# alibaba/EasyRec

Hardware: AMD Instinct MI355X
Metric: global examples/sec + emb HBM GB/s, DeepFM Criteo-shape b4096 @1/2/4/8 GPU (higher is better)
Workload: dtype f32; 1 GPU; DeepFM synthetic Criteo: deepfm_criteo.config (39 features: 26 hashed x 1000000 rows + 13 projected, D=16 deep + D=1 wide, batch 4096 per GPU, optimizer adam_optimizer (lazy dense decay, closed-form replay), ids zipf, hipGraph replay); timed steps cycle over 256 distinct device-generated batches after 1024 untimed pre-conditioning steps; global_batch=4096, parallelism=single GPU

## Files before the change

### easyrec_amd/csrc/er_embedding.hip

```cpp
#include <algorithm>
#include <cmath>
#include <cstring>
#include <vector>

#include "er_common.h"
#include "er_gemm_core.h"
#include "er_dense_tail.h"
#include "er_decay.h"
#include "er_grad_finish.h"

namespace er {

constexpr uint32_t kInvalidKey = 0xFFFFFFFFu;

__host__ __device__ __forceinline__ void lane_geom(int dim, int& V, int& G) {
  V = (dim % 4 == 0) ? 4 : 1;
  const int n = dim / V;
  G = 1;
  while (G < n) G <<= 1;
}

__device__ __forceinline__ int find_lookup(const int32_t* __restrict__ blk_start, int n, int bid) {
  int lo = 0, hi = n;
  while (hi - lo > 1) {
// ... 1266 lines not shown
  float* s_all = smem;
  for (int i = tid; i < kProjParts * (dim + 1); i += kBlock)
    s_all[i] = __hip_atomic_load(all + i, __ATOMIC_RELAXED, __HIP_MEMORY_SCOPE_SYSTEM);
  __syncthreads();
  if (tid >= G || !col_ok) return;
  float g[V];
#pragma unroll
  for (int j = 0; j < V; ++j) g[j] = 0.f;
  float n_valid = 0.f;
  for (int k = 0; k < kProjParts; ++k) {
#pragma unroll
    for (int j = 0; j < V; ++j) g[j] = g[j] + s_all[k * (dim + 1) + c + j];
    n_valid = n_valid + s_all[k * (dim + 1) + dim];
  }
  if (n_valid == 0.f) return;
  const ReduceOut ro{0, nullptr, nullptr, nullptr, nullptr, 0};
  finish_run<V>(a.tab, ma.opt_kind, ma.hyper, ro, static_cast<uint32_t>(d.key_base), 0, sub, c, dim, g, a.aux);
  if (dbg && tid == 0) dbg[1] = wall_clock64();
}

#ifndef ER_OWN_WAVES
#define ER_OWN_WAVES 4
#endif
__device__ __forceinline__ void own_block(int bid, const OwnMulti& ma, float* smem) {
  if (bid < ma.start[ma.n]) {
    int i = 0;
    while (i + 1 < ma.n && bid >= ma.start[i + 1]) ++i;
    const OwnArgs& a = ma.a[i];
    if (a.V == 4) own_tile_body<4>(bid - ma.start[i], ma, a, smem);
    else own_tile_body<1>(bid - ma.start[i], ma, a, smem);
    return;
  }
  const int pb = bid - ma.start[ma.n];
  int i = 0;
  while (i + 1 < ma.n && pb >= ma.proj_start[i + 1]) ++i;
  const OwnArgs& a = ma.a[i];
  if (a.V == 4) own_proj_body<4>(pb - ma.proj_start[i], ma, a, smem);
  else own_proj_body<1>(pb - ma.proj_start[i], ma, a, smem);
}

__global__ void __launch_bounds__(kBlock) __attribute__((amdgpu_waves_per_eu(ER_OWN_WAVES)))
emb_bwd_own_kernel(OwnMulti ma) {
  extern __shared__ __attribute__((aligned(16))) float smem[];
  own_block(blockIdx.x, ma, smem);
}

__global__ void __launch_bounds__(kBlock) __attribute__((amdgpu_waves_per_eu(ER_OWN_WAVES)))
emb_bwd_own_wgrad_kernel(OwnMulti ma, GroupedArgs ga, int n_gemm, int n_own, LossTailArgs lt) {
  extern __shared__ __attribute__((aligned(16))) float smem[];
  const int bid = blockIdx.x;
  if (bid < n_gemm) {
    const GroupedCoords c = grouped_coords(ga, bid);
    if (c.split < 0) return;
    gemm_f32_block<false, false>(ga.p[c.p], c.tile, c.split, smem, c.plain);
    return;
  }
  if (bid - n_gemm < n_own) own_block(bid - n_gemm, ma, smem);
  else loss_tail_body<kBlock>(lt, smem);
}

struct CatchHeadsArgs {
  const uint32_t* ukeys_seg;
  const uint32_t* seg_count;
  const int64_t* ent_base;
  int n_lookups;
  int64_t n;
  RowUpdate tab;
  DecayAux aux;
  int dim, G, V;
  const uint32_t* extra_keys;
  int n_extra;
  int cap_shift;
};
struct CatchHeadsMulti {
  int n;
  int start[kMaxMulti + 1];
  const er_opt_hyper* hyper;
  CatchHeadsArgs a[kMaxMulti];
};

template <int V>
__device__ __forceinline__ void catch_up_row(const CatchHeadsArgs& a, uint32_t key, int c, int32_t t, float eps) {
  const int32_t s_begin = a.tab.ls(key) + 1;
  if (s_begin >= t) return;
  const int64_t off = a.tab.off(key, c);
  float var[V], m[V], v[V];
  ld_vec<V>(m, a.tab.m + off);
  ld_vec<V>(v, a.tab.v + off);
  bool live = false;
#pragma unroll
  for (int j = 0; j < V; ++j) live = live || (m[j] != 0.f) || (v[j] != 0.f);
  if (live) {
    ld_vec<V>(var, a.tab.var + off);
    replay_closed<V>(var, m, v, a.aux, s_begin, t, eps);
    st_vec<V>(a.tab.var + off, var);
    st_vec<V>(a.tab.m + off, m);
    st_vec<V>(a.tab.v + off, v);
  }
  if (c == 0) a.tab.ls(key) = t - 1;
}

template <int V>
__device__ __forceinline__ void catch_heads_body(int bid, const CatchHeadsArgs& a, const er_opt_hyper* __restrict__ hyper) {
  __shared__ int s_base[kOwnMaxLookups + 1], s_cnt[kOwnMaxLookups + 1];
  const int tid = threadIdx.x;
  const int ppb = kBlock / a.G;
  const int c = (tid % a.G) * V;
// ... 3408 lines not shown
```

### easyrec_amd/csrc/er_gemm.hip

```cpp
#include "er_gemm_core.h"

namespace er {

template <bool A_KC, bool B_KC>
__global__ void __launch_bounds__(kBlock)
gemm_f32_kernel(GemmArgs g) {
  __shared__ __attribute__((aligned(16))) float lds[2 * 2 * kOpTile];
  gemm_f32_block<A_KC, B_KC>(g, blockIdx.x, blockIdx.z, lds);
}

template <bool A_KC, bool B_KC>
__global__ void __launch_bounds__(kBlock)
gemm_f32_bn_bwd_kernel(GemmArgs g) {
  __shared__ __attribute__((aligned(16))) float lds[2 * 2 * kOpTile];
  gemm_f32_block<A_KC, B_KC, true>(g, blockIdx.x, 0, lds);
}

template <bool A_KC, bool B_KC, int XEPI>
__global__ void __launch_bounds__(kBlock)
gemm_f32_cross_kernel(GemmArgs g, er_gemm_epilogue xe) {
  __shared__ __attribute__((aligned(16))) float lds[2 * 2 * kOpTile];
  gemm_f32_block<A_KC, B_KC, false, XEPI>(g, blockIdx.x, 0, lds, false, &xe);
}

template <bool A_KC, bool B_KC, int DIN>
__global__ void __launch_bounds__(kBlock)
gemm_f32_din_kernel(GemmArgs g, DinGen d) {
  __shared__ __attribute__((aligned(16))) float lds[2 * 2 * kOpTile];
  gemm_f32_block<A_KC, B_KC, false, 0, DIN>(g, blockIdx.x, blockIdx.z, lds, false, nullptr, &d);
}

__global__ void __launch_bounds__(kBlock)
gemm_f32_bna_kernel(GemmArgs g, BnA b) {
  __shared__ __attribute__((aligned(16))) float lds[2 * 2 * kOpTile];
  __shared__ __attribute__((aligned(16))) float coef[4 * kBnAMaxK];
  bna_load_coef(b, g.K, coef);
  __syncthreads();
  gemm_f32_block<true, false, false, 0, 3>(g, blockIdx.x, 0, lds, false, nullptr, nullptr, &b, coef);
}

template <int NC>
__global__ void __launch_bounds__(kBlock)
gemv_bna_kernel(const float* __restrict__ x, int ldx, int M, int K, BnA b, const float* __restrict__ W, int ldw,
                const float* __restrict__ bias, float* __restrict__ C, int ldc, int lpr) {
  constexpr int R = 4;
  const int rpb = kBlock / lpr;
  const int lr = threadIdx.x % lpr;
  const int r0 = (static_cast<int>(blockIdx.x) * R) * rpb + threadIdx.x / lpr;
  const bool bn = b.mean != nullptr;
  float acc[R][NC];
#pragma unroll
  for (int u = 0; u < R; ++u)
#pragma unroll
    for (int n = 0; n < NC; ++n) acc[u][n] = 0.f;
  for (int c = lr; c < K / 4; c += lpr) {
    const int k = 4 * c;
    f32x4v xv[R];
#pragma unroll
    for (int u = 0; u < R; ++u) {
      int row = r0 + u * rpb;
      row = row < M ? row : M - 1;
      xv[u] = *reinterpret_cast<const f32x4v*>(x + static_cast<int64_t>(row) * ldx + k);
    }
    float w[4][NC];
#pragma unroll
    for (int j = 0; j < 4; ++j)
#pragma unroll
      for (int n = 0; n < NC; ++n) w[j][n] = W[static_cast<int64_t>(k + j) * ldw + n];
// ... 309 lines not shown
  __shared__ __attribute__((aligned(16))) short Bs[BN * kBf16SH];
  const GroupedCoords c = grouped_coords(ga, blockIdx.x);
  if (c.split < 0) return;
  gemm_bf16_block<A_KC, B_KC>(ga.p[c.p], c.tile, c.split, As, Bs, c.plain);
}


template <int VEC>
__global__ void __launch_bounds__(kBlock)
gemm_splitk_reduce_kernel(const float* __restrict__ ws, int64_t mn, int N, int splits, const float* __restrict__ bias,
                          float* __restrict__ C, int ldc, int accumulate) {
  splitk_reduce_elems<VEC>(ws, mn, N, splits, bias, C, ldc, accumulate,
                           (static_cast<int64_t>(blockIdx.x) * kBlock + threadIdx.x) * VEC);
}


template <int VEC>
__global__ void __launch_bounds__(kBlock)
gemm_splitk_reduce_grouped_kernel(GroupedReduceArgs ra) {
  splitk_reduce_grouped_block<VEC>(ra, blockIdx.x);
}

}

namespace {

float* g_gemm_ws = nullptr;
size_t g_gemm_ws_floats = 0;

int ensure_ws(size_t floats, float** out) {
  if (floats > g_gemm_ws_floats) {
    if (g_gemm_ws) (void)hipFree(g_gemm_ws);
    g_gemm_ws = nullptr;
    g_gemm_ws_floats = 0;
    ER_CHECK_HIP(hipMalloc(&g_gemm_ws, floats * sizeof(float)));
    g_gemm_ws_floats = floats;
  }
  *out = g_gemm_ws;
  return 0;
}

template <bool BF16>
int launch_gemm(int layout, er::GemmArgs& a, hipStream_t s) {
  const int64_t n_tiles = er::ceil_div(a.N, er::BN) * er::ceil_div(a.M, er::BM);
  dim3 grid(static_cast<unsigned>(n_tiles), 1, static_cast<unsigned>(a.splits));
  dim3 block(er::kBlock);
#define ER_LAUNCH_GEMM(KERNEL)                                                   \
  switch (layout) {                                                              \
    case ER_GEMM_NN: hipLaunchKernelGGL((KERNEL<true, false>), grid, block, 0, s, a); break;  \
    case ER_GEMM_NT: hipLaunchKernelGGL((KERNEL<true, true>), grid, block, 0, s, a); break;   \
    case ER_GEMM_TN: hipLaunchKernelGGL((KERNEL<false, false>), grid, block, 0, s, a); break; \
    default: er::set_error("er_gemm: unknown layout %d", layout); return 2;     \
  }
  if (BF16) {
    ER_LAUNCH_GEMM(er::gemm_bf16_kernel)
  } else if (a.bn.partial) {
    ER_LAUNCH_GEMM(er::gemm_f32_bn_bwd_kernel)
  } else {
    ER_LAUNCH_GEMM(er::gemm_f32_kernel)
  }
#undef ER_LAUNCH_GEMM
  ER_LAUNCH_CHECK();
  return 0;
}

int choose_splits(int M, int N, int K, int ktile) {
  const int64_t tiles = er::ceil_div(M, er::BM) * er::ceil_div(N, er::BN);
  if (tiles >= 256 || K < 1024) return 1;
  int64_t s = 512 / tiles;
  const int64_t max_by_k = K / (4 * ktile);
  if (s > max_by_k) s = max_by_k;
  if (s > 64) s = 64;
  return s < 1 ? 1 : static_cast<int>(s);
}

template <bool BF16>
int gemm_entry(int layout, int M, int N, int K, const float* A, int lda, const float* B, int ldb, float* C, int ldc,
               const float* bias, int accumulate, float* col_stats, er_stream_t stream, const char* who,
               const er::BnBwdEpi* bn = nullptr) {
  ER_REQUIRE(A && B && C && M > 0 && N > 0 && K > 0, "%s: bad arguments", who);
  ER_REQUIRE(layout >= ER_GEMM_NN && layout <= ER_GEMM_TN, "%s: unknown layout %d", who, layout);
  const int min_lda = (layout == ER_GEMM_TN) ? M : K;
  const int min_ldb = (layout == ER_GEMM_NT) ? K : N;
  ER_REQUIRE(lda >= min_lda && ldb >= min_ldb && ldc >= N, "%s: leading dimension too small", who);
  hipStream_t s = er::as_stream(stream);
  constexpr int ktile = BF16 ? er::BK16 : er::BK32;
  er::GemmArgs a;
  a.A = A; a.B = B; a.C = C; a.bias = bias;
  a.M = M; a.N = N; a.K = K; a.lda = lda; a.ldb = ldb; a.ldc = ldc;
  a.accumulate = accumulate;
  a.col_stats = col_stats;
  if (bn) {
    a.bn = *bn;
    if (a.bn.n_src == 0) { a.bn.col0 = 0; a.bn.n_src = N; }
  }
  a.splits = (col_stats || bn) ? 1 : choose_splits(M, N, K, ktile);
  ER_REQUIRE(!(col_stats && accumulate), "%s: column statistics need a plain (non-accumulating) output", who);
  a.k_per_split = static_cast<int>(er::ceil_div(er::ceil_div(K, a.splits), ktile)) * ktile;
  a.splits = static_cast<int>(er::ceil_div(K, a.k_per_split));
  if (a.splits > 1) {
    float* ws;
    if (int rc = ensure_ws(static_cast<size_t>(a.splits) * M * N, &ws)) return rc;
    a.C = ws;
    if (int rc = launch_gemm<BF16>(layout, a, s)) return rc;
    const int64_t mn = static_cast<int64_t>(M) * N;
    if (N % 4 == 0 && ldc % 4 == 0 && (reinterpret_cast<uintptr_t>(C) & 15) == 0) {
      hipLaunchKernelGGL(er::gemm_splitk_reduce_kernel<4>, dim3(static_cast<unsigned>(er::ceil_div(mn / 4, er::kBlock))),
                         dim3(er::kBlock), 0, s, ws, mn, N, a.splits, bias, C, ldc, accumulate);
    } else {
      hipLaunchKernelGGL(er::gemm_splitk_reduce_kernel<1>, dim3(static_cast<unsigned>(er::ceil_div(mn, er::kBlock))),
                         dim3(er::kBlock), 0, s, ws, mn, N, a.splits, bias, C, ldc, accumulate);
    }
    ER_LAUNCH_CHECK();
// ... 517 lines not shown
```

### easyrec_amd/csrc/er_gemm_core.h

```cpp
#pragma once
#include "er_common.h"

namespace er {

typedef float f32x16 __attribute__((ext_vector_type(16)));
typedef float f32x4v __attribute__((ext_vector_type(4)));
typedef short bf16x8 __attribute__((ext_vector_type(8)));
typedef short bf16x4 __attribute__((ext_vector_type(4)));

constexpr int BM = 64, BN = 64;
constexpr int BK32 = 32;
constexpr int BK16 = 32;

struct BnBwdEpi {
  const float* z = nullptr;
  const float* zbias = nullptr;
  const float* y = nullptr;
  const float* mean = nullptr;
  const float* invstd = nullptr;
  int ld = 0, use_bn = 0, act = 0;
  float* partial = nullptr;
  int col0 = 0, n_src = 0;
  const float* gamma = nullptr;
  int dz_out = 0;
};

struct GemmArgs {
  const float* A;
  const float* B;
  float* C;
  const float* bias;
  int M, N, K;
  int lda, ldb, ldc;
  int accumulate;
  int k_per_split;
  int splits;
  float* col_stats;
  BnBwdEpi bn;
  float* fz_y = nullptr;
  float* fz_save = nullptr;
  float fz_eps = 0.f;
};
constexpr int kEpiFrozenBn = 7;
constexpr int kEpiFrozenDz = 8;

template <bool K_CONTIG>
__device__ __forceinline__ f32x4v load4(const float* __restrict__ P, int ld, int mn, int k, int MN, int K,
                                        bool vec_ok) {
  f32x4v v = {0.f, 0.f, 0.f, 0.f};
  if (K_CONTIG) {
    if (mn >= MN) return v;
    const float* p = P + static_cast<int64_t>(mn) * ld + k;
    if (vec_ok && k + 3 < K) {
// ... 80 lines not shown
    if (row < M) { const float d = out[r] - mean; m2 += d * d; }
  }
  const float on = __shfl_xor(n, 32, 64), om = __shfl_xor(mean, 32, 64), o2 = __shfl_xor(m2, 32, 64);
  float an = khalf ? on : n, am = khalf ? om : mean, a2 = khalf ? o2 : m2;
  chan_merge(an, am, a2, khalf ? n : on, khalf ? mean : om, khalf ? m2 : o2);
  __syncthreads();
  float* slot = lds + (wn * 32 + (lane & 31)) * 3;
  if (wm == 1 && khalf == 0) { slot[0] = an; slot[1] = am; slot[2] = a2; }
  __syncthreads();
  if (wm == 0 && khalf == 0 && col < N) {
    chan_merge(an, am, a2, slot[0], slot[1], slot[2]);
    float* o = out_tile + static_cast<int64_t>(col) * 3;
    o[0] = an; o[1] = am; o[2] = a2;
  }
}

__device__ __forceinline__ void tile_bn_bwd_partial(const f32x16& acc, const BnBwdEpi& e, const float (&py)[16],
                                                    const float (&pz)[16], int row_base, int M, int col, int N, int wm,
                                                    int wn, int lane, float* lds, int ty) {
  const int khalf = lane >> 5;
  float sg = 0.f, sgx = 0.f;
  const bool col_ok = col >= 0 && col < N;
  if (col_ok) {
    float bv = e.zbias ? e.zbias[col] : 0.f;
    float mu = e.use_bn ? e.mean[col] : 0.f;
    float is = e.use_bn ? e.invstd[col] : 0.f;
    pin(bv); pin(mu); pin(is);
#pragma unroll
    for (int r = 0; r < 16; ++r) {
      const int row = row_base + (r & 3) + 8 * (r >> 2) + 4 * khalf;
      if (row < M) {
        float g = acc[r];
        if (e.act == ER_ACT_RELU && !(py[r] > 0.f)) g = 0.f;
        sg = sg + g;
        if (e.use_bn) sgx = sgx + g * ((pz[r] + bv - mu) * is);
      }
    }
  }
  const float og = __shfl_xor(sg, 32, 64), ogx = __shfl_xor(sgx, 32, 64);
  const float a = (khalf ? og : sg) + (khalf ? sg : og);
  const float ax = (khalf ? ogx : sgx) + (khalf ? sgx : ogx);
  __syncthreads();
  float* slot = lds + (wn * 32 + (lane & 31)) * 2;
  if (wm == 1 && khalf == 0) { slot[0] = a; slot[1] = ax; }
  __syncthreads();
  if (wm == 0 && khalf == 0 && col_ok) {
    float* p = e.partial + (static_cast<int64_t>(ty) * N + col) * 2;
    p[0] = a + slot[0];
    p[1] = ax + slot[1];
  }
}

constexpr int SK = BK32 + 4;
constexpr int kOpTile = BM * SK;

template <bool KC>
__device__ __forceinline__ void unit_pos(int tid, int i, int& row, int& k) {
  if (KC) {
    const int u = tid + i * kBlock;
    row = u >> 3;
    k = (u & 7) * 4;
  } else {
    row = (tid >> 4) * 4;
    k = (tid & 15) + 16 * i;
  }
}

template <bool KC>
__device__ __forceinline__ void fetch_tile(const float* __restrict__ P, int ld, int mn0, int MN, int k0, int kend,
                                           int K, int tid, f32x4v (&r)[2]) {
#pragma unroll
  for (int i = 0; i < 2; ++i) {
    int row, k;
    unit_pos<KC>(tid, i, row, k);
    int mn = mn0 + row;
    k += k0;
    if (KC) {
      const int kpad = (K + 3) & ~3;
      mn = mn < MN ? mn : MN - 1;
      k = k < kpad - 4 ? k : kpad - 4;
      r[i] = *reinterpret_cast<const f32x4v*>(P + static_cast<int64_t>(mn) * ld + k);
    } else {
      const int mnpad = (MN + 3) & ~3;
      mn = mn < mnpad - 4 ? mn : mnpad - 4;
      k = k < kend ? k : kend - 1;
      r[i] = *reinterpret_cast<const f32x4v*>(P + static_cast<int64_t>(k) * ld + mn);
    }
  }
}

template <bool KC>
__device__ __forceinline__ void fetch_tile_generic(const float* __restrict__ P, int ld, int mn0, int MN, int k0,
                                                   int kend, int tid, f32x4v (&r)[2]) {
#pragma unroll
  for (int i = 0; i < 2; ++i) {
    int row, k;
    unit_pos<KC>(tid, i, row, k);
    const int mn = mn0 + row;
    k += k0;
#pragma unroll
    for (int j = 0; j < 4; ++j) {
      bool ok;
      int64_t at;
      if (KC) {
        ok = mn < MN && k + j < kend;
        at = static_cast<int64_t>(mn < MN ? mn : MN - 1) * ld + (k + j < kend ? k + j : kend - 1);
      } else {
        ok = mn + j < MN && k < kend;
        at = static_cast<int64_t>(k < kend ? k : kend - 1) * ld + (mn + j < MN ? mn + j : MN - 1);
      }
      const float v = P[at];
      r[i][j] = ok ? v : 0.f;
    }
  }
}

template <bool KC>
__device__ __forceinline__ void stage_tile(float* __restrict__ S, int tid, const f32x4v (&r)[2], bool interior, int mn0,
                                           int MN, int k0, int kend) {
#pragma unroll
  for (int i = 0; i < 2; ++i) {
    int row, k;
    unit_pos<KC>(tid, i, row, k);
    f32x4v v = r[i];
    if (!interior) {
#pragma unroll
      for (int j = 0; j < 4; ++j) {
        const bool ok = KC ? (mn0 + row < MN && k0 + k + j < kend) : (mn0 + row + j < MN && k0 + k < kend);
        if (!ok) v[j] = 0.f;
      }
    }
    if (KC) {
      *reinterpret_cast<f32x4v*>(&S[row * SK + k]) = v;
    } else {
#pragma unroll
      for (int j = 0; j < 4; ++j) S[(row + j) * SK + k] = v[j];
    }
  }
}

struct DinGen {
  const float* q;
  const float* h;
  int ldq, ldh, L, E;
  uint32_t inv_L;
  uint32_t inv_E;
  float* dh;
  int lddh, accumulate_dh;
  float* dq_partial;
  int slots;
};
__device__ __forceinline__ int din_div_L(const DinGen& d, int row) {
  return static_cast<int>((static_cast<uint64_t>(static_cast<uint32_t>(row)) * d.inv_L) >> 32);
}
__device__ __forceinline__ f32x4v din_combine(int seg, const f32x4v& qv, const f32x4v& hv) {
  const bool odd = (seg & 1) != 0, hi = (seg & 2) != 0;
  f32x4v v;
#pragma unroll
  for (int j = 0; j < 4; ++j) {
    const float sub = qv[j] - hv[j], mul = qv[j] * hv[j];
    const float lo_v = odd ? hv[j] : qv[j];
    const float hi_v = odd ? mul : sub;
    v[j] = hi ? hi_v : lo_v;
  }
  return v;
}
struct DinPre {
  const float* qp[2];
  const float* hp[2];
  int off[2];
  int seg[2];
};
template <bool KC>
__device__ __forceinline__ void din_prepare(const DinGen& d, int mn0, int MN, int tid, DinPre& p) {
#pragma unroll
  for (int i = 0; i < 2; ++i) {
    int row, k;
    unit_pos<KC>(tid, i, row, k);
    p.off[i] = k;
    if (KC) {
      int r = mn0 + row;
      r = r < MN ? r : MN - 1;
      const int b = din_div_L(d, r);
      p.qp[i] = d.q + static_cast<int64_t>(b) * d.ldq;
      p.hp[i] = d.h + static_cast<int64_t>(r) * d.ldh;
      p.seg[i] = 0;
    } else {
      int c = mn0 + row;
      c = c < MN - 4 ? c : MN - 4;
      const int seg = static_cast<int>((static_cast<uint64_t>(static_cast<uint32_t>(c)) * d.inv_E) >> 32);
      p.seg[i] = seg;
      p.qp[i] = d.q + (c - seg * d.E);
      p.hp[i] = d.h + (c - seg * d.E);
    }
  }
}
template <bool KC>
__device__ __forceinline__ void fetch_din(const DinGen& d, const DinPre& p, int k0, int kend, int K, f32x4v (&rh)[2],
                                          f32x4v (&rq)[2]) {
#pragma unroll
  for (int i = 0; i < 2; ++i) {
    if (KC) {
      int c = k0 + p.off[i];
      c = c < K - 4 ? c : K - 4;
      const int seg = static_cast<int>((static_cast<uint64_t>(static_cast<uint32_t>(c)) * d.inv_E) >> 32);
      const int j = c - seg * d.E;
      rq[i] = *reinterpret_cast<const f32x4v*>(p.qp[i] + j);
      rh[i] = *reinterpret_cast<const f32x4v*>(p.hp[i] + j);
    } else {
      int r = k0 + p.off[i];
      r = r < kend ? r : kend - 1;
      const int b = din_div_L(d, r);
      rq[i] = *reinterpret_cast<const f32x4v*>(p.qp[i] + static_cast<int64_t>(b) * d.ldq);
      rh[i] = *reinterpret_cast<const f32x4v*>(p.hp[i] + static_cast<int64_t>(r) * d.ldh);
    }
  }
}
template <bool KC>
__device__ __forceinline__ void combine_din(const DinGen& d, const DinPre& p, int k0, int K, f32x4v (&rh)[2],
                                            const f32x4v (&rq)[2]) {
#pragma unroll
  for (int i = 0; i < 2; ++i) {
    int seg = p.seg[i];
    if (KC) {
      int c = k0 + p.off[i];
      c = c < K - 4 ? c : K - 4;
      seg = static_cast<int>((static_cast<uint64_t>(static_cast<uint32_t>(c)) * d.inv_E) >> 32);
    }
    rh[i] = din_combine(seg, rq[i], rh[i]);
  }
}
__device__ __forceinline__ void fetch_tile_din_perm(const float* __restrict__ P, int ld, int tx, int E, int k0, int kend, int K,
                                                    int tid, f32x4v (&r)[2]) {
#pragma unroll
  for (int i = 0; i < 2; ++i) {
    int row, k;
    unit_pos<true>(tid, i, row, k);
    const int n = (row >> 4) * E + tx * 16 + (row & 15);
    k += k0;
    const int kpad = (K + 3) & ~3;
    k = k < kpad - 4 ? k : kpad - 4;
    r[i] = *reinterpret_cast<const f32x4v*>(P + static_cast<int64_t>(n) * ld + k);
  }
}

struct BnA {
  const float* mean;
  const float* invstd;
  const float* gamma;
  const float* beta;
  int act;
  float* y;
  int ldy;
};
constexpr int kBnAMaxK = 256;
__device__ __forceinline__ void bna_load_coef(const BnA& b, int K, float* __restrict__ coef) {
  for (int k = threadIdx.x; k < ((K + 3) & ~3); k += kBlock) {
    const bool in = k < K;
    f32x4v c = {in ? b.mean[k] : 0.f, in ? b.invstd[k] : 0.f, (in && b.gamma) ? b.gamma[k] : 1.f, (in && b.beta) ? b.beta[k] : 0.f};
    *reinterpret_cast<f32x4v*>(coef + 4 * k) = c;
  }
}
__device__ __forceinline__ void bna_apply(const BnA& b, const float* __restrict__ coef, int tid, int m0, int M, int k0, int K,
                                          bool store, f32x4v (&r)[2]) {
  int kk = k0 + (tid & 7) * 4;
  const int kpad = (K + 3) & ~3;
  kk = kk < kpad - 4 ? kk : kpad - 4;
  f32x4v c[4];
#pragma unroll
  for (int j = 0; j < 4; ++j) c[j] = *reinterpret_cast<const f32x4v*>(coef + 4 * (kk + j));
#pragma unroll
  for (int i = 0; i < 2; ++i) {
    f32x4v v;
#pragma unroll
    for (int j = 0; j < 4; ++j) {
      float t = (r[i][j] - c[j][0]) * c[j][1];
      t = t * c[j][2] + c[j][3];
      if (b.act == ER_ACT_RELU) t = t > 0.f ? t : 0.f;
      v[j] = t;
    }
    r[i] = v;
    const int row = m0 + ((tid + i * kBlock) >> 3);
    if (store && row < M && k0 + (tid & 7) * 4 < K)
      *reinterpret_cast<f32x4v*>(b.y + static_cast<int64_t>(row) * b.ldy + kk) = v;
  }
}

template <bool A_KC, bool B_KC, bool BN_EPI = false, int XEPI = 0, int DIN = 0>
__device__ __forceinline__ void gemm_f32_block(const GemmArgs& g, int bx, int bz, float* __restrict__ lds,
                                               bool plain_tiles = false, const er_gemm_epilogue* xe = nullptr,
                                               const DinGen* dg = nullptr, const BnA* ba = nullptr,
                                               const float* __restrict__ coef = nullptr) {
  const int tid = threadIdx.x;
  const int lane = tid & 63, wave = tid >> 6;
  const int wm = wave >> 1, wn = wave & 1;
  int tx, ty;
  tile_coords(bx, static_cast<int>(ceil_div(g.N, BN)), static_cast<int>(ceil_div(g.M, BM)), tx, ty, plain_tiles);
  const int m0 = ty * BM, n0 = tx * BN;
  const int kbeg = bz * g.k_per_split;
  int kend = kbeg + g.k_per_split;
  if (kend > g.K) kend = g.K;
  const int T = (kend - kbeg + BK32 - 1) / BK32;
  float py[16], pz[16];
  if (BN_EPI && g.bn.partial != nullptr) {
    int c = n0 + wn * 32 + (lane & 31) - g.bn.col0;
    c = c < 0 ? 0 : (c < g.bn.n_src ? c : g.bn.n_src - 1);
#pragma unroll
    for (int r = 0; r < 16; ++r) {
      int row = m0 + wm * 32 + (r & 3) + 8 * (r >> 2) + 4 * (lane >> 5);
      row = row < g.M ? row : g.M - 1;
      const int64_t i = static_cast<int64_t>(row) * g.bn.ld + c;
      py[r] = g.bn.y[i];
      pz[r] = g.bn.z[i];
    }
  }
  float qa[XEPI ? 16 : 1], qb[XEPI ? 16 : 1], qc[XEPI == ER_EPI_CROSS_BWD ? 16 : 1], qd[XEPI == ER_EPI_CROSS_BWD ? 16 : 1],
      qe[XEPI == ER_EPI_CROSS_BWD ? 16 : 1], qf[XEPI == ER_EPI_CROSS_BWD ? 16 : 1];
  if (XEPI && XEPI != kEpiFrozenBn && XEPI != kEpiFrozenDz) {
    int c = n0 + wn * 32 + (lane & 31);
    c = c < g.N ? c : g.N - 1;
    const bool with_diag = xe->diag != 0.f;
#pragma unroll
    for (int r = 0; r < 16; ++r) {
      int row = m0 + wm * 32 + (r & 3) + 8 * (r >> 2) + 4 * (lane >> 5);
      row = row < g.M ? row : g.M - 1;
      const int64_t rr = row;
      if (XEPI == ER_EPI_CROSS_FWD) {
        qa[r] = xe->x0[rr * xe->ld_x0 + c];
        qb[r] = xe->xl[rr * xe->ld_xl + c];
      } else {
        qa[r] = xe->dout[rr * xe->ld_dout + c];
        qb[r] = with_diag ? xe->du_in[rr * xe->ld_du_in + c] : 0.f;
        if (xe->prev_u) {
          qc[r] = xe->x0[rr * xe->ld_x0 + c];
          qd[r] = xe->prev_u[rr * xe->ld_prev_u + c];
          qe[r] = with_diag ? xe->xl[rr * xe->ld_xl + c] : 0.f;
          qf[r] = xe->accumulate_dx0 ? xe->dx0[rr * xe->ld_dx0 + c] : 0.f;
        }
      }
    }
  }
  const bool a_vec = (g.lda % 4 == 0) && ((reinterpret_cast<uintptr_t>(g.A) & 15) == 0);
  const bool b_vec = (g.ldb % 4 == 0) && ((reinterpret_cast<uintptr_t>(g.B) & 15) == 0);
  const bool rows_full = (m0 + BM <= g.M) && (n0 + BN <= g.N);
  const bool rows_all = m0 + BM <= g.M;
  const int col = n0 + wn * 32 + (lane & 31);
  float bv = 0.f;
  if (g.bias && g.splits == 1) bv = g.bias[col < g.N ? col : g.N - 1];

  f32x16 acc;
#pragma unroll
  for (int i = 0; i < 16; ++i) acc[i] = 0.f;
  const int khalf = lane >> 5;
  const int fa = (wm * 32 + (lane & 31)) * SK + khalf * 16;
  const int fb = kOpTile + (wn * 32 + (lane & 31)) * SK + khalf * 16;
  auto contract = [&](const float* base, f32x4v (&a)[4], f32x4v (&b)[4]) {
#pragma unroll
    for (int q = 0; q < 4; ++q)
#pragma unroll
      for (int i = 0; i < 4; ++i) acc = __builtin_amdgcn_mfma_f32_32x32x2f32(a[q][i], b[q][i], acc, 0, 0, 0);
  };
  auto read_frags = [&](const float* base, f32x4v (&a)[4], f32x4v (&b)[4]) {
#pragma unroll
    for (int q = 0; q < 4; ++q) {
      a[q] = *reinterpret_cast<const f32x4v*>(base + fa + 4 * q);
      b[q] = *reinterpret_cast<const f32x4v*>(base + fb + 4 * q);
    }
  };

  if (DIN || (a_vec && b_vec)) {
    f32x4v ra0[2], rb0[2], ra1[2], rb1[2];
    f32x4v rq0[2], rq1[2];
    DinPre dpre;
    if (DIN == 1) din_prepare<A_KC>(*dg, m0, g.M, tid, dpre);
    auto fetch = [&](f32x4v (&ra)[2], f32x4v (&rb)[2], f32x4v (&rq)[2], int t) {
      const int k0 = kbeg + (t < T ? t : T - 1) * BK32;
      if (DIN == 1) fetch_din<A_KC>(*dg, dpre, k0, kend, g.K, ra, rq);
      else fetch_tile<A_KC>(g.A, g.lda, m0, g.M, k0, kend, g.K, tid, ra);
      if (DIN == 2) fetch_tile_din_perm(g.B, g.ldb, tx, dg->E, k0, kend, g.K, tid, rb);
      else if (DIN == 3 && !b_vec) fetch_tile_generic<B_KC>(g.B, g.ldb, n0, g.N, k0, kend, tid, rb);
      else fetch_tile<B_KC>(g.B, g.ldb, n0, g.N, k0, kend, g.K, tid, rb);
    };
    auto stage = [&](int buf, f32x4v (&ra)[2], const f32x4v (&rb)[2], const f32x4v (&rq)[2], int t) {
      const int k0 = kbeg + t * BK32;
      const bool interior = rows_full && (k0 + BK32 <= kend);
      if (DIN == 1) combine_din<A_KC>(*dg, dpre, kbeg + (t < T ? t : T - 1) * BK32, g.K, ra, rq);
      if (DIN == 3) bna_apply(*ba, coef, tid, m0, g.M, kbeg + (t < T ? t : T - 1) * BK32, g.K, tx == 0 && t < T && ba->y != nullptr, ra);
      stage_tile<A_KC>(lds + buf * 2 * kOpTile, tid, ra, interior, m0, g.M, k0, kend);
      stage_tile<B_KC>(lds + buf * 2 * kOpTile + kOpTile, tid, rb, interior, n0, g.N, k0, kend);
    };
    auto step = [&](int buf, f32x4v (&fa_)[2], f32x4v (&fb_)[2], f32x4v (&fq_)[2], f32x4v (&sa)[2], f32x4v (&sb)[2],
                    f32x4v (&sq)[2], int t) {
      const float* base = lds + buf * 2 * kOpTile;
      fetch(fa_, fb_, fq_, t + 2);
#pragma unroll
      for (int q = 0; q < 3; ++q) {
        const f32x4v a = *reinterpret_cast<const f32x4v*>(base + fa + 4 * q);
        const f32x4v b = *reinterpret_cast<const f32x4v*>(base + fb + 4 * q);
#pragma unroll
        for (int i = 0; i < 4; ++i) acc = __builtin_amdgcn_mfma_f32_32x32x2f32(a[i], b[i], acc, 0, 0, 0);
      }
      stage(buf ^ 1, sa, sb, sq, t + 1);
      {
        const f32x4v a = *reinterpret_cast<const f32x4v*>(base + fa + 12);
        const f32x4v b = *reinterpret_cast<const f32x4v*>(base + fb + 12);
#pragma unroll
        for (int i = 0; i < 4; ++i) acc = __builtin_amdgcn_mfma_f32_32x32x2f32(a[i], b[i], acc, 0, 0, 0);
      }
      __syncthreads();
    };
    fetch(ra0, rb0, rq0, 0);
    fetch(ra1, rb1, rq1, 1);
    stage(0, ra0, rb0, rq0, 0);
    __syncthreads();
    for (int t = 0; t < T; t += 2) {
      step(0, ra0, rb0, rq0, ra1, rb1, rq1, t);
      step(1, ra1, rb1, rq1, ra0, rb0, rq0, t + 1);
    }
  } else {
    f32x4v ra[2], rb[2];
    for (int t = 0; t < T; ++t) {
      const int k0 = kbeg + t * BK32;
      fetch_tile_generic<A_KC>(g.A, g.lda, m0, g.M, k0, kend, tid, ra);
      fetch_tile_generic<B_KC>(g.B, g.ldb, n0, g.N, k0, kend, tid, rb);
      stage_tile<A_KC>(lds, tid, ra, true, m0, g.M, k0, kend);
      stage_tile<B_KC>(lds + kOpTile, tid, rb, true, n0, g.N, k0, kend);
      __syncthreads();
      f32x4v a[4], b[4];
      read_frags(lds, a, b);
      contract(lds, a, b);
      __syncthreads();
    }
  }
  const int row0 = m0 + wm * 32 + 4 * khalf;
  pin(bv);
  float out[16];
#pragma unroll
  for (int r = 0; r < 16; ++r) out[r] = acc[r] + bv;
  if (g.col_stats)
    tile_col_stats(out, m0 + wm * 32, g.M, col, g.N, wm, wn, lane, lds,
                   g.col_stats + static_cast<int64_t>(ty) * g.N * 3);
  if (BN_EPI && g.bn.partial != nullptr) {
    tile_bn_bwd_partial(acc, g.bn, py, pz, m0 + wm * 32, g.M, col < g.N ? col - g.bn.col0 : -1, g.bn.n_src, wm, wn, lane, lds, ty);
    if (XEPI == kEpiFrozenDz && g.bn.dz_out) {
      if (col >= g.N) return;
      const float ga = g.bn.gamma ? g.bn.gamma[col] : 1.f;
      const float is = g.bn.invstd[col];
      float dz[16];
#pragma unroll
      for (int r = 0; r < 16; ++r) {
        float gg = out[r];
        if (g.bn.act == ER_ACT_RELU && !(py[r] > 0.f)) gg = 0.f;
        dz[r] = ga * is * gg;
      }
      pin(dz);
      store16(g.C + static_cast<int64_t>(row0) * g.ldc + col, g.ldc, row0, g.M, rows_all, dz);
      return;
    }
  }
  if (DIN == 2) {
    const DinGen& d = *dg;
    constexpr int kD = 65;
    float* D = lds;
    float* Es = lds + 64 * kD;
    __syncthreads();
#pragma unroll
    for (int r = 0; r < 16; ++r) {
      const int rl = wm * 32 + (r & 3) + 8 * (r >> 2) + 4 * khalf;
      D[rl * kD + wn * 32 + (lane & 31)] = acc[r];
    }
// ... 283 lines not shown
```

Measured before the change: 14.12 million examples/s.

## Pin GEMM main-loop instruction schedule with sched barriers for small grids

Adds a PINNED variant of the f32 GEMM block that interleaves the global fetches, LDS staging and LDS fragment reads between individual MFMA instructions, using sched_barrier to stop the compiler reordering them. It also peels an interior loop that skips bounds masking. The variant is used for small GEMM launches (at most 256 workgroups) and for the fused backward wgrad kernel, where it is meant to hide memory latency when occupancy is low. Risks are higher register pressure and a fixed schedule that could be worse than the compiler's own. The bn_bwd pinned kernel also gets a launch-bounds occupancy hint.

```diff
diff --git a/easyrec_amd/csrc/er_embedding.hip b/easyrec_amd/csrc/er_embedding.hip
--- a/easyrec_amd/csrc/er_embedding.hip
+++ b/easyrec_amd/csrc/er_embedding.hip
@@ -1342,7 +1342,7 @@
   if (bid < n_gemm) {
     const GroupedCoords c = grouped_coords(ga, bid);
     if (c.split < 0) return;
-    gemm_f32_block<false, false>(ga.p[c.p], c.tile, c.split, smem, c.plain);
+    gemm_f32_block<false, false, false, 0, 0, true>(ga.p[c.p], c.tile, c.split, smem, c.plain);
     return;
   }
   if (bid - n_gemm < n_own) own_block(bid - n_gemm, ma, smem);
diff --git a/easyrec_amd/csrc/er_gemm.hip b/easyrec_amd/csrc/er_gemm.hip
--- a/easyrec_amd/csrc/er_gemm.hip
+++ b/easyrec_amd/csrc/er_gemm.hip
@@ -14,6 +14,21 @@
 gemm_f32_bn_bwd_kernel(GemmArgs g) {
   __shared__ __attribute__((aligned(16))) float lds[2 * 2 * kOpTile];
   gemm_f32_block<A_KC, B_KC, true>(g, blockIdx.x, 0, lds);
+}
+
+struct PinnedOrder {};
+template <bool A_KC, bool B_KC>
+__global__ void __launch_bounds__(kBlock)
+gemm_f32_kernel(GemmArgs g, PinnedOrder) {
+  __shared__ __attribute__((aligned(16))) float lds[2 * 2 * kOpTile];
+  gemm_f32_block<A_KC, B_KC, false, 0, 0, true>(g, blockIdx.x, blockIdx.z, lds);
+}
+
+template <bool A_KC, bool B_KC>
+__global__ void __launch_bounds__(kBlock, 4)
+gemm_f32_bn_bwd_kernel(GemmArgs g, PinnedOrder) {
+  __shared__ __attribute__((aligned(16))) float lds[2 * 2 * kOpTile];
+  gemm_f32_block<A_KC, B_KC, true, 0, 0, true>(g, blockIdx.x, 0, lds);
 }
 
 template <bool A_KC, bool B_KC, int XEPI>
@@ -429,13 +444,22 @@
     case ER_GEMM_TN: hipLaunchKernelGGL((KERNEL<false, false>), grid, block, 0, s, a); break; \
     default: er::set_error("er_gemm: unknown layout %d", layout); return 2;     \
   }
+#define ER_LAUNCH_GEMM_PINNED(KERNEL)                                              \
+  switch (layout) {                                                              \
+    case ER_GEMM_NN: hipLaunchKernelGGL((KERNEL<true, false>), grid, block, 0, s, a, er::PinnedOrder()); break;  \
+    case ER_GEMM_NT: hipLaunchKernelGGL((KERNEL<true, true>), grid, block, 0, s, a, er::PinnedOrder()); break;   \
+    case ER_GEMM_TN: hipLaunchKernelGGL((KERNEL<false, false>), grid, block, 0, s, a, er::PinnedOrder()); break; \
+    default: er::set_error("er_gemm: unknown layout %d", layout); return 2;     \
+  }
+  const bool pinned = n_tiles * a.splits <= er::kPinnedMaxWorkgroups;
   if (BF16) {
     ER_LAUNCH_GEMM(er::gemm_bf16_kernel)
   } else if (a.bn.partial) {
-    ER_LAUNCH_GEMM(er::gemm_f32_bn_bwd_kernel)
+    if (pinned) { ER_LAUNCH_GEMM_PINNED(er::gemm_f32_bn_bwd_kernel) } else { ER_LAUNCH_GEMM(er::gemm_f32_bn_bwd_kernel) }
   } else {
-    ER_LAUNCH_GEMM(er::gemm_f32_kernel)
-  }
+    if (pinned) { ER_LAUNCH_GEMM_PINNED(er::gemm_f32_kernel) } else { ER_LAUNCH_GEMM(er::gemm_f32_kernel) }
+  }
+#undef ER_LAUNCH_GEMM_PINNED
 #undef ER_LAUNCH_GEMM
   ER_LAUNCH_CHECK();
   return 0;
diff --git a/easyrec_amd/csrc/er_gemm_core.h b/easyrec_amd/csrc/er_gemm_core.h
--- a/easyrec_amd/csrc/er_gemm_core.h
+++ b/easyrec_amd/csrc/er_gemm_core.h
@@ -1,4 +1,6 @@
 #pragma once
+#include <type_traits>
+
 #include "er_common.h"
 
 namespace er {
@@ -185,6 +187,7 @@
 }
 
 constexpr int SK = BK32 + 4;
+constexpr int kPinnedMaxWorkgroups = 256;
 constexpr int kOpTile = BM * SK;
 
 template <bool KC>
@@ -200,76 +203,79 @@
 }
 
 template <bool KC>
-__device__ __forceinline__ void fetch_tile(const float* __restrict__ P, int ld, int mn0, int MN, int k0, int kend,
-                                           int K, int tid, f32x4v (&r)[2]) {
-#pragma unroll
-  for (int i = 0; i < 2; ++i) {
-    int row, k;
-    unit_pos<KC>(tid, i, row, k);
-    int mn = mn0 + row;
-    k += k0;
+__device__ __forceinline__ void fetch_unit(const float* __restrict__ P, int ld, int mn0, int MN, int k0, int kend,
+                                           int K, int tid, int i, f32x4v& r) {
+  int row, k;
+  unit_pos<KC>(tid, i, row, k);
+  int mn = mn0 + row;
+  k += k0;
+  if (KC) {
+    const int kpad = (K + 3) & ~3;
+    mn = mn < MN ? mn : MN - 1;
+    k = k < kpad - 4 ? k : kpad - 4;
+    r = *reinterpret_cast<const f32x4v*>(P + static_cast<int64_t>(mn) * ld + k);
+  } else {
+    const int mnpad = (MN + 3) & ~3;
+    mn = mn < mnpad - 4 ? mn : mnpad - 4;
+    k = k < kend ? k : kend - 1;
+    r = *reinterpret_cast<const f32x4v*>(P + static_cast<int64_t>(k) * ld + mn);
+  }
+}
+
+template <bool KC>
+__device__ __forceinline__ void fetch_unit_generic(const float* __restrict__ P, int ld, int mn0, int MN, int k0,
+                                                   int kend, int tid, int i, f32x4v& r) {
+  int row, k;
+  unit_pos<KC>(tid, i, row, k);
+  const int mn = mn0 + row;
+  k += k0;
+#pragma unroll
+  for (int j = 0; j < 4; ++j) {
+    bool ok;
+    int64_t at;
     if (KC) {
-      const int kpad = (K + 3) & ~3;
-      mn = mn < MN ? mn : MN - 1;
-      k = k < kpad - 4 ? k : kpad - 4;
-      r[i] = *reinterpret_cast<const f32x4v*>(P + static_cast<int64_t>(mn) * ld + k);
+      ok = mn < MN && k + j < kend;
+      at = static_cast<int64_t>(mn < MN ? mn : MN - 1) * ld + (k + j < kend ? k + j : kend - 1);
     } else {
-      const int mnpad = (MN + 3) & ~3;
-      mn = mn < mnpad - 4 ? mn : mnpad - 4;
-      k = k < kend ? k : kend - 1;
-      r[i] = *reinterpret_cast<const f32x4v*>(P + static_cast<int64_t>(k) * ld + mn);
-    }
-  }
-}
-
+      ok = mn + j < MN && k < kend;
+      at = static_cast<int64_t>(k < kend ? k : kend - 1) * ld + (mn + j < MN ? mn + j : MN - 1);
+    }
+    const float v = P[at];
+    r[j] = ok ? v : 0.f;
+  }
+}
 template <bool KC>
 __device__ __forceinline__ void fetch_tile_generic(const float* __restrict__ P, int ld, int mn0, int MN, int k0,
                                                    int kend, int tid, f32x4v (&r)[2]) {
 #pragma unroll
-  for (int i = 0; i < 2; ++i) {
-    int row, k;
-    unit_pos<KC>(tid, i, row, k);
-    const int mn = mn0 + row;
-    k += k0;
+  for (int i = 0; i < 2; ++i) fetch_unit_generic<KC>(P, ld, mn0, MN, k0, kend, tid, i, r[i]);
+}
+
+template <bool KC>
+__device__ __forceinline__ void stage_unit(float* __restrict__ S, int tid, int i, const f32x4v& r, bool interior, int mn0,
+                                           int MN, int k0, int kend) {
+  int row, k;
+  unit_pos<KC>(tid, i, row, k);
+  f32x4v v = r;
+  if (!interior) {
 #pragma unroll
     for (int j = 0; j < 4; ++j) {
-      bool ok;
-      int64_t at;
-      if (KC) {
-        ok = mn < MN && k + j < kend;
-        at = static_cast<int64_t>(mn < MN ? mn : MN - 1) * ld + (k + j < kend ? k + j : kend - 1);
-      } else {
-        ok = mn + j < MN && k < kend;
-        at = static_cast<int64_t>(k < kend ? k : kend - 1) * ld + (mn + j < MN ? mn + j : MN - 1);
-      }
-      const float v = P[at];
-      r[i][j] = ok ? v : 0.f;
-    }
-  }
-}
-
+      const bool ok = KC ? (mn0 + row < MN && k0 + k + j < kend) : (mn0 + row + j < MN && k0 + k < kend);
+      if (!ok) v[j] = 0.f;
+    }
+  }
+  if (KC) {
+    *reinterpret_cast<f32x4v*>(&S[row * SK + k]) = v;
+  } else {
+#pragma unroll
+    for (int j = 0; j < 4; ++j) S[(row + j) * SK + k] = v[j];
+  }
+}
 template <bool KC>
 __device__ __forceinline__ void stage_tile(float* __restrict__ S, int tid, const f32x4v (&r)[2], bool interior, int mn0,
                                            int MN, int k0, int kend) {
 #pragma unroll
-  for (int i = 0; i < 2; ++i) {
-    int row, k;
-    unit_pos<KC>(tid, i, row, k);
-    f32x4v v = r[i];
-    if (!interior) {
-#pragma unroll
-      for (int j = 0; j < 4; ++j) {
-        const bool ok = KC ? (mn0 + row < MN && k0 + k + j < kend) : (mn0 + row + j < MN && k0 + k < kend);
-        if (!ok) v[j] = 0.f;
-      }
-    }
-    if (KC) {
-      *reinterpret_cast<f32x4v*>(&S[row * SK + k]) = v;
-    } else {
-#pragma unroll
-      for (int j = 0; j < 4; ++j) S[(row + j) * SK + k] = v[j];
-    }
-  }
+  for (int i = 0; i < 2; ++i) stage_unit<KC>(S, tid, i, r[i], interior, mn0, MN, k0, kend);
 }
 
 struct DinGen {
@@ -329,24 +335,21 @@
   }
 }
 template <bool KC>
-__device__ __forceinline__ void fetch_din(const DinGen& d, const DinPre& p, int k0, int kend, int K, f32x4v (&rh)[2],
-                                          f32x4v (&rq)[2]) {
-#pragma unroll
-  for (int i = 0; i < 2; ++i) {
-    if (KC) {
-      int c = k0 + p.off[i];
-      c = c < K - 4 ? c : K - 4;
-      const int seg = static_cast<int>((static_cast<uint64_t>(static_cast<uint32_t>(c)) * d.inv_E) >> 32);
-      const int j = c - seg * d.E;
-      rq[i] = *reinterpret_cast<const f32x4v*>(p.qp[i] + j);
-      rh[i] = *reinterpret_cast<const f32x4v*>(p.hp[i] + j);
-    } else {
-      int r = k0 + p.off[i];
-      r = r < kend ? r : kend - 1;
-      const int b = din_div_L(d, r);
-      rq[i] = *reinterpret_cast<const f32x4v*>(p.qp[i] + static_cast<int64_t>(b) * d.ldq);
-      rh[i] = *reinterpret_cast<const f32x4v*>(p.hp[i] + static_cast<int64_t>(r) * d.ldh);
-    }
+__device__ __forceinline__ void fetch_din_unit(const DinGen& d, const DinPre& p, int k0, int kend, int K, int i,
+                                               f32x4v (&rh)[2], f32x4v (&rq)[2]) {
+  if (KC) {
+    int c = k0 + p.off[i];
+    c = c < K - 4 ? c : K - 4;
+    const int seg = static_cast<int>((static_cast<uint64_t>(static_cast<uint32_t>(c)) * d.inv_E) >> 32);
+    const int j = c - seg * d.E;
+    rq[i] = *reinterpret_cast<const f32x4v*>(p.qp[i] + j);
+    rh[i] = *reinterpret_cast<const f32x4v*>(p.hp[i] + j);
+  } else {
+    int r = k0 + p.off[i];
+    r = r < kend ? r : kend - 1;
+    const int b = din_div_L(d, r);
+    rq[i] = *reinterpret_cast<const f32x4v*>(p.qp[i] + static_cast<int64_t>(b) * d.ldq);
+    rh[i] = *reinterpret_cast<const f32x4v*>(p.hp[i] + static_cast<int64_t>(r) * d.ldh);
   }
 }
 template <bool KC>
@@ -363,18 +366,15 @@
     rh[i] = din_combine(seg, rq[i], rh[i]);
   }
 }
-__device__ __forceinline__ void fetch_tile_din_perm(const float* __restrict__ P, int ld, int tx, int E, int k0, int kend, int K,
-                                                    int tid, f32x4v (&r)[2]) {
-#pragma unroll
-  for (int i = 0; i < 2; ++i) {
-    int row, k;
-    unit_pos<true>(tid, i, row, k);
-    const int n = (row >> 4) * E + tx * 16 + (row & 15);
-    k += k0;
-    const int kpad = (K + 3) & ~3;
-    k = k < kpad - 4 ? k : kpad - 4;
-    r[i] = *reinterpret_cast<const f32x4v*>(P + static_cast<int64_t>(n) * ld + k);
-  }
+__device__ __forceinline__ void fetch_unit_din_perm(const float* __restrict__ P, int ld, int tx, int E, int k0, int kend, int K,
+                                                    int tid, int i, f32x4v& r) {
+  int row, k;
+  unit_pos<true>(tid, i, row, k);
+  const int n = (row >> 4) * E + tx * 16 + (row & 15);
+  k += k0;
+  const int kpad = (K + 3) & ~3;
+  k = k < kpad - 4 ? k : kpad - 4;
+  r = *reinterpret_cast<const f32x4v*>(P + static_cast<int64_t>(n) * ld + k);
 }
 
 struct BnA {
@@ -419,7 +419,7 @@
   }
 }
 
-template <bool A_KC, bool B_KC, bool BN_EPI = false, int XEPI = 0, int DIN = 0>
+template <bool A_KC, bool B_KC, bool BN_EPI = false, int XEPI = 0, int DIN = 0, bool PINNED = false>
 __device__ __forceinline__ void gemm_f32_block(const GemmArgs& g, int bx, int bz, float* __restrict__ lds,
                                                bool plain_tiles = false, const er_gemm_epilogue* xe = nullptr,
                                                const DinGen* dg = nullptr, const BnA* ba = nullptr,
@@ -506,24 +506,77 @@
     f32x4v rq0[2], rq1[2];
     DinPre dpre;
     if (DIN == 1) din_prepare<A_KC>(*dg, m0, g.M, tid, dpre);
+    auto fetch_part = [&](f32x4v (&ra)[2], f32x4v (&rb)[2], f32x4v (&rq)[2], int t, int part) {
+      const int k0 = kbeg + (t < T ? t : T - 1) * BK32;
+      const int i = part & 1;
+      if (part < 2) {
+        if (DIN == 1) fetch_din_unit<A_KC>(*dg, dpre, k0, kend, g.K, i, ra, rq);
+        else fetch_unit<A_KC>(g.A, g.lda, m0, g.M, k0, kend, g.K, tid, i, ra[i]);
+      } else {
+        if (DIN == 2) fetch_unit_din_perm(g.B, g.ldb, tx, dg->E, k0, kend, g.K, tid, i, rb[i]);
+        else if (DIN == 3 && !b_vec) fetch_unit_generic<B_KC>(g.B, g.ldb, n0, g.N, k0, kend, tid, i, rb[i]);
+        else fetch_unit<B_KC>(g.B, g.ldb, n0, g.N, k0, kend, g.K, tid, i, rb[i]);
+      }
+    };
+    auto stage_part = [&](int buf, f32x4v (&ra)[2], const f32x4v (&rb)[2], const f32x4v (&rq)[2], int t, int part,
+                          bool interior) {
+      const int k0 = kbeg + t * BK32;
+      const int i = part & 1;
+      if (part == 0) {
+        if (DIN == 1) combine_din<A_KC>(*dg, dpre, kbeg + (t < T ? t : T - 1) * BK32, g.K, ra, rq);
+        if (DIN == 3) bna_apply(*ba, coef, tid, m0, g.M, kbeg + (t < T ? t : T - 1) * BK32, g.K, tx == 0 && t < T && ba->y != nullptr, ra);
+      }
+      if (part < 2) stage_unit<A_KC>(lds + buf * 2 * kOpTile, tid, i, ra[i], interior, m0, g.M, k0, kend);
+      else stage_unit<B_KC>(lds + buf * 2 * kOpTile + kOpTile, tid, i, rb[i], interior, n0, g.N, k0, kend);
+    };
     auto fetch = [&](f32x4v (&ra)[2], f32x4v (&rb)[2], f32x4v (&rq)[2], int t) {
-      const int k0 = kbeg + (t < T ? t : T - 1) * BK32;
-      if (DIN == 1) fetch_din<A_KC>(*dg, dpre, k0, kend, g.K, ra, rq);
-      else fetch_tile<A_KC>(g.A, g.lda, m0, g.M, k0, kend, g.K, tid, ra);
-      if (DIN == 2) fetch_tile_din_perm(g.B, g.ldb, tx, dg->E, k0, kend, g.K, tid, rb);
-      else if (DIN == 3 && !b_vec) fetch_tile_generic<B_KC>(g.B, g.ldb, n0, g.N, k0, kend, tid, rb);
-      else fetch_tile<B_KC>(g.B, g.ldb, n0, g.N, k0, kend, g.K, tid, rb);
+#pragma unroll
+      for (int part = 0; part < 4; ++part) fetch_part(ra, rb, rq, t, part);
     };
     auto stage = [&](int buf, f32x4v (&ra)[2], const f32x4v (&rb)[2], const f32x4v (&rq)[2], int t) {
-      const int k0 = kbeg + t * BK32;
-      const bool interior = rows_full && (k0 + BK32 <= kend);
-      if (DIN == 1) combine_din<A_KC>(*dg, dpre, kbeg + (t < T ? t : T - 1) * BK32, g.K, ra, rq);
-      if (DIN == 3) bna_apply(*ba, coef, tid, m0, g.M, kbeg + (t < T ? t : T - 1) * BK32, g.K, tx == 0 && t < T && ba->y != nullptr, ra);
-      stage_tile<A_KC>(lds + buf * 2 * kOpTile, tid, ra, interior, m0, g.M, k0, kend);
-      stage_tile<B_KC>(lds + buf * 2 * kOpTile + kOpTile, tid, rb, interior, n0, g.N, k0, kend);
+      const bool interior = rows_full && (kbeg + t * BK32 + BK32 <= kend);
+#pragma unroll
+      for (int part = 0; part < 4; ++part) stage_part(buf, ra, rb, rq, t, part, interior);
     };
-    auto step = [&](int buf, f32x4v (&fa_)[2], f32x4v (&fb_)[2], f32x4v (&fq_)[2], f32x4v (&sa)[2], f32x4v (&sb)[2],
-                    f32x4v (&sq)[2], int t) {
+#define ER_PIN() __builtin_amdgcn_sched_barrier(0)
+    auto step = [&](auto masked, int buf, f32x4v (&fa_)[2], f32x4v (&fb_)[2], f32x4v (&fq_)[2], f32x4v (&sa)[2],
+                    f32x4v (&sb)[2], f32x4v (&sq)[2], int t) {
+      constexpr bool kInterior = !decltype(masked)::value;
+      const float* base = lds + buf * 2 * kOpTile;
+      f32x4v a[2], b[2];
+      a[0] = *reinterpret_cast<const f32x4v*>(base + fa);
+      b[0] = *reinterpret_cast<const f32x4v*>(base + fb);
+#pragma unroll
+      for (int q = 0; q < 4; ++q) {
+        const f32x4v aq = a[q & 1], bq = b[q & 1];
+#pragma unroll
+        for (int i = 0; i < 4; ++i) {
+          if (q == 3 && i == 3) {
+            ER_PIN();
+            __syncthreads();
+            ER_PIN();
+          }
+          acc = __builtin_amdgcn_mfma_f32_32x32x2f32(aq[i], bq[i], acc, 0, 0, 0);
+          if (q == 3) continue;
+          ER_PIN();
+          if (i == 0) {
+            a[(q + 1) & 1] = *reinterpret_cast<const f32x4v*>(base + fa + 4 * (q + 1));
+            b[(q + 1) & 1] = *reinterpret_cast<const f32x4v*>(base + fb + 4 * (q + 1));
+          }
+          if (q < 2 && i < 2) fetch_part(fa_, fb_, fq_, t + 2, 2 * q + i);
+          if (q == 2 && i == 0) {
+            ER_PIN();
+            stage_part(buf ^ 1, sa, sb, sq, t + 1, 0, kInterior);
+            stage_part(buf ^ 1, sa, sb, sq, t + 1, 1, kInterior);
+          }
+          if (q == 2 && (i == 1 || i == 2)) stage_part(buf ^ 1, sa, sb, sq, t + 1, i + 1, kInterior);
+          ER_PIN();
+        }
+      }
+    };
+#undef ER_PIN
+    auto step_free = [&](int buf, f32x4v (&fa_)[2], f32x4v (&fb_)[2], f32x4v (&fq_)[2], f32x4v (&sa)[2], f32x4v (&sb)[2],
+                         f32x4v (&sq)[2], int t) {
       const float* base = lds + buf * 2 * kOpTile;
       fetch(fa_, fb_, fq_, t + 2);
 #pragma unroll
@@ -546,9 +599,23 @@
     fetch(ra1, rb1, rq1, 1);
     stage(0, ra0, rb0, rq0, 0);
     __syncthreads();
-    for (int t = 0; t < T; t += 2) {
-      step(0, ra0, rb0, rq0, ra1, rb1, rq1, t);
-      step(1, ra1, rb1, rq1, ra0, rb0, rq0, t + 1);
+    int t = 0;
+    if (!PINNED) {
+      for (; t < T; t += 2) {
+        step_free(0, ra0, rb0, rq0, ra1, rb1, rq1, t);
+        step_free(1, ra1, rb1, rq1, ra0, rb0, rq0, t + 1);
+      }
+    } else {
+      if (rows_full) {
+        for (; kbeg + (t + 3) * BK32 <= kend; t += 2) {
+          step(std::false_type(), 0, ra0, rb0, rq0, ra1, rb1, rq1, t);
+          step(std::false_type(), 1, ra1, rb1, rq1, ra0, rb0, rq0, t + 1);
+        }
+      }
+      for (; t < T; t += 2) {
+        step(std::true_type(), 0, ra0, rb0, rq0, ra1, rb1, rq1, t);
+        step(std::true_type(), 1, ra1, rb1, rq1, ra0, rb0, rq0, t + 1);
+      }
     }
   } else {
     f32x4v ra[2], rb[2];
```

Measured after the change: 14.57 million examples/s, median of 6. 3.2% higher.
